# nygenome/lancet

Measured on AMD Instinct MI355X. Metric: assembled windows/sec (whole node), 600bp windows, self-tuning k, synthetic T/N, higher is better.
Workload: dtype u64; 1 GPU; chr22-scan proxy: 32768 windows/GPU x 600 bp, stride 100, 30x tumor / 30x normal, 2x150 bp, k=11..101, active-region-off; windows_per_gpu=32768, reads_per_gpu=5895305, records_rank0_contig=22477, slots_in_flight=4080, batches_in_flight=2, windows_first_graph_in_lds=32768, graphs_built_ahead=2147, graphs_taken_from_pool=2037, windows_rerun_worst_case_tier=0

## Files before the change

lancet_amd/csrc/kernels.h:

```cpp
#pragma once
#include "wave.h"
#include "layout.h"
#include "../../include/lancet_engine.h"

#ifndef LANCET_WG
#define LANCET_WG 64
#endif
#ifdef LANCET_FAT
#define LC_QLANES LC_FAT_LANES
#define LC_PF_G 6
#define LC_QSTAGE (3 * LC_FAT_LANES)
#else
#define LC_QLANES LANCET_WG
#define LC_QSTAGE LC_STAGE
#endif

enum {
  EV_PROCESS = 1, EV_REPEAT_REF, EV_NEAR_REF, EV_READS, EV_STATS, EV_MARKREF, EV_LOWCOV, EV_CLEANDEAD,
  EV_COMPRESS, EV_CC, EV_CCID, EV_CCEND, EV_TRIM, EV_AMBIG_SRC, EV_NOMATCH_SRC, EV_AMBIG_SNK, EV_NOMATCH_SNK,
  EV_CYCLE, EV_TIPS_ROUND, EV_TIPS_REMOVED, EV_LINKS, EV_LOOKREP, EV_MISSING, EV_SEARCH, EV_NEAR_QRY,
  EV_DFSLIMIT, EV_PATH, EV_TS, EV_PATH_END, EV_EKA_END, EV_FOUND, EV_END
};

struct WalkState { int nts, last_col, code; };
// ... 3596 lines not shown
      dir = dir_dest(ED_DIR(e));
    }
  }
  return len;
}
DEVNI int path_string_wg(Ctx &c, int n) {
  LC_GLOBAL Work &W = *LC_CTX(c).W; LC_WS &S = LC_SREF(c);
  const int K = S.K;
  const int dcap = 7 * ((int)LC_CTX(c).C->max_w + 2);
  if (2 * (n + 1) > dcap || n < 2) { WG_LANE0 { S.ps_len = path_string(c, n); } return wg_bcast(&S.ps_len); }
  if (n <= 64) {
    volatile LC_LDS uint8_t *lb = &S.lbytes[0];
    volatile LC_LDS uint32_t *loff = (volatile LC_LDS uint32_t *)lb, *llen = loff + 66, *lslo = llen + 64, *lshi = lslo + 64;
    volatile LC_LDS uint8_t *ldir = (volatile LC_LDS uint8_t *)(lshi + 64);
    static_assert(4 * (66 + 3 * 64) + 64 <= (int)sizeof(S.lbytes), "path nodes staged in LDS");
    WG_LANE0 { S.ps_first = 0x7FFFFFFF; }
    WG_FOR(i, n) {
      const uint32_t nd = W.pnodes[i];
      const uint32_t pe = W.pedges[i == 0 ? 1 : i];
      LC_GLOBAL const uint32_t *g = (LC_GLOBAL const uint32_t *)&W.gr[nd];
      const uint32_t fl = g[0]; const lc_u4 h1 = ldg4(g + 20);
      const uint32_t e = W.gr[pe >> 4].edges[pe & 15u];
      const bool sp = (fl & NF_SPECIAL) != 0;
      if (!sp) dev_atomic_min((LC_LDS uint32_t *)&S.ps_first, (uint32_t)i);
      ldir[i] = (uint8_t)(i == 0 ? dir_start(ED_DIR(e)) : dir_dest(ED_DIR(e)));
      lslo[i] = h1.z; lshi[i] = h1.w; llen[i] = sp ? 0xFFFFFFFFu : h1.w - h1.z;
    }
    WG_SYNC();
    const int f = wg_uniform(S.ps_first);
    WG_FOR(i, n + 1) {
      uint32_t sum = 0;
      for (int j = 0; j < i; ++j) { const uint32_t L = llen[j]; if (L != 0xFFFFFFFFu) sum += (j == f ? L : L - (uint32_t)(K - 1)); }
      loff[i] = sum;
    }
    WG_SYNC();
    const int plen = (int)wg_uniform((int)loff[n]);
    if (plen > (int)LC_CTX(c).C->path_cap) { WG_LANE0 { OVF(c); } return 0; }
    WG_FOR(x, plen) {
      int lo = 0, hi = n - 1;
      while (lo < hi) { const int mid = (lo + hi + 1) >> 1; if ((int)loff[mid] <= x) lo = mid; else hi = mid - 1; }
      while (lo > 0 && loff[lo + 1] == loff[lo]) --lo;
      const uint32_t slo = lslo[lo], shi = lshi[lo];
      const uint32_t j = (uint32_t)(x - (int)loff[lo]) + (lo == f ? 0u : (uint32_t)(K - 1));
      const uint32_t d = (ldir[lo] == (uint8_t)'R') ? (W.seq[shi - 1 - j] ^ 3u) : W.seq[slo + j];
      W.pdesc[x] = d; W.pseq[x] = (uint8_t)SD_BASE(d);
    }
    WG_SYNC();
    return plen;
  }
  LC_GLOBAL uint32_t *off = (LC_GLOBAL uint32_t *)W.dp, *pdir = off + (n + 1);
  WG_LANE0 { S.ps_first = 0x7FFFFFFF; off[n] = 0; }
  WG_FOR(i, n) {
    const uint32_t nd = W.pnodes[i];
    if (!(W.gr[nd].flags & NF_SPECIAL)) dev_atomic_min((LC_LDS uint32_t *)&S.ps_first, (uint32_t)i);
    const uint32_t pe = W.pedges[i == 0 ? 1 : i];
    const uint32_t e = W.gr[pe >> 4].edges[pe & 15u];
    pdir[i] = (uint32_t)(i == 0 ? dir_start(ED_DIR(e)) : dir_dest(ED_DIR(e)));
  }
  WG_SYNC();
  const int f = wg_uniform(S.ps_first);
  WG_FOR(i, n) {
    const uint32_t nd = W.pnodes[i];
    const int L = n_len(c, nd);
    off[i] = (W.gr[nd].flags & NF_SPECIAL) ? 0u : (uint32_t)(i == f ? L : L - (K - 1));
  }
  WG_SYNC();
  wg_scan(off, n + 1, S, S.part2);
  const int plen = (int)wg_uniform((int)S.part2[LANCET_WG]);
  if (plen > (int)LC_CTX(c).C->path_cap) { WG_LANE0 { OVF(c); } return 0; }
  WG_FOR(x, plen) {
    int lo = 0, hi = n - 1;
    while (lo < hi) { const int mid = (lo + hi + 1) >> 1; if ((int)off[mid] <= x) lo = mid; else hi = mid - 1; }
    while (lo > 0 && off[lo + 1] == off[lo]) --lo;
    const uint32_t nd = W.pnodes[lo];
    const uint32_t slo = W.gr[nd].seq_lo, shi = W.gr[nd].seq_hi;
    const uint32_t j = (uint32_t)(x - (int)off[lo]) + (lo == f ? 0u : (uint32_t)(K - 1));
    const uint32_t d = (pdir[lo] == (uint32_t)'R') ? (W.seq[shi - 1 - j] ^ 3u) : W.seq[slo + j];
    W.pdesc[x] = d; W.pseq[x] = (uint8_t)SD_BASE(d);
  }
  WG_SYNC();
  return plen;
}
DEV bool status_cnt_T(const Ctx &c, uint32_t n) {
  double pr = (double)LC_CTX(c).W->gr[n].nkmT / (double)LC_CTX(c).W->gr[n].nkm;
  return pr > 0.8;
}

#define LC_TB(i, j, n) ((size_t)((i) + (j)) * (size_t)((n) + 1) + (size_t)(i))
DEV void align_fill_arrays(Ctx &c, LC_GLOBAL const uint8_t *Sx, int n, LC_GLOBAL const uint8_t *Tx, int m) {
  LC_GLOBAL Work &W = *LC_CTX(c).W;
  const int A = (int)LC_CTX(c).C->max_w + 2;
  int32_t *Mb[3] = {W.dp, W.dp + A, W.dp + 2 * A};
  int32_t *Xb[2] = {W.dp + 3 * A, W.dp + 4 * A};
  int32_t *Yb[2] = {W.dp + 5 * A, W.dp + 6 * A};
  WG_FOR(j, m + 1) { W.tb[LC_TB(0, j, n)] = (uint8_t)((j == 0 ? 3 : 2) | (0 << 2) | (2 << 4)); }
  WG_FOR(i, n + 1) { if (i > 0) W.tb[LC_TB(i, 0, n)] = (uint8_t)(1 | (2 << 2) | (0 << 4)); }
  WG_LANE0 { Mb[0][0] = 0; Mb[1][0] = -9; Xb[1][0] = -9; Mb[1][1] = -9; Yb[1][1] = -9; }
  WG_SYNC();
  for (int d = 2; d <= n + m; ++d) {
    int32_t *Mc = Mb[d % 3], *Mp = Mb[(d + 2) % 3], *Mpp = Mb[(d + 1) % 3];
    int32_t *Xc = Xb[d & 1], *Xp = Xb[(d + 1) & 1], *Yc = Yb[d & 1], *Yp = Yb[(d + 1) & 1];
    int ilo = d - m; if (ilo < 1) ilo = 1;
    int ihi = d - 1; if (ihi > n) ihi = n;
    WG_FOR(t, ihi - ilo + 1) {
      int i = ilo + t, j = d - i;
      int xa = Xp[i - 1] + (-1), xb = Mp[i - 1] + (-8);
      int xs, xt; if (xa > xb) { xs = xa; xt = 1; } else { xs = xb; xt = 0; }
      int ya = Yp[i] + (-1), yb = Mp[i] + (-8);
      int ys, yt; if (ya > yb) { ys = ya; yt = 1; } else { ys = yb; yt = 0; }
      int ms = Mpp[i - 1] + (Sx[i - 1] == Tx[j - 1] ? 2 : -4), mt = 0;
      if (xs > ms) { ms = xs; mt = 1; }
      if (ys > ms) { ms = ys; mt = 2; }
      Mc[i] = ms; Xc[i] = xs; Yc[i] = ys;
      W.tb[LC_TB(i, j, n)] = (uint8_t)(mt | (xt << 2) | (yt << 4));
    }
    WG_LANE0 {
      if (d <= m) { Mc[0] = -8 - d; Xc[0] = -8 - d; }
      if (d <= n) { Mc[d] = -8 - d; Yc[d] = -8 - d; }
    }
    WG_SYNC();
  }
}
#ifndef LANCET_WAVE_EMU
template <int GMAX>
DEVNI void align_fill_g(Ctx &c, LC_GLOBAL const uint8_t *Sx, int n, LC_GLOBAL const uint8_t *Tx, int m) {
  static_assert(LANCET_WG == 64, "one wave per window");
  LC_GLOBAL Work &W = *LC_CTX(c).W;
  if (threadIdx.x == 0) LC_SREF(c).al_band = 0;
  const int lane = (int)threadIdx.x;
  if (lane < 64) {
  for (int j = lane; j < m + 1; j += 64) W.tb[LC_TB(0, j, n)] = (uint8_t)((j == 0 ? 3 : 2) | (0 << 2) | (2 << 4));
  for (int i = lane + 1; i < n + 1; i += 64) W.tb[LC_TB(i, 0, n)] = (uint8_t)(1 | (2 << 2) | (0 << 4));
  const int G = (n + 63) / 64;
  int A[GMAX], Bv[GMAX], sg[GMAX];
  auto lo16 = [](int v) -> int { return (int)(short)(v & 0xFFFF); };
  auto hi16 = [](int v) -> int { return v >> 16; };
  auto pack = [](int lo, int hi) -> int { return (lo & 0xFFFF) | (hi << 16); };
#pragma unroll
  for (int g = 0; g < GMAX; ++g) {
    int i = g * 64 + lane + 1;
    A[g] = pack(-8 - i, 0);
    Bv[g] = pack(-8 - i, (i - 1 == 0) ? 0 : -8 - (i - 1));
    sg[g] = (i <= n) ? (int)Sx[i - 1] : 255;
  }
  for (int t = 2; t <= n + m; ++t) {
#pragma unroll
    for (int gg = 0; gg < GMAX; ++gg) {
      const int g = GMAX - 1 - gg;
      if (g < G) {
        int i = g * 64 + lane + 1, j = t - i;
        int nb = __shfl_up(A[g], 1);
        if (g > 0) { int e = __shfl(A[g > 0 ? g - 1 : 0], 63); if (lane == 0) nb = e; }
        else if (lane == 0) nb = pack(-8 - j, -8 - j);
        int nbM = lo16(nb), nbX = hi16(nb);
        bool active = (i <= n) && (j >= 1) && (j <= m);
        int bv = Bv[g];
        if (active) {
          int xa = nbX - 1, xb = nbM - 8;
          int xs, xt; if (xa > xb) { xs = xa; xt = 1; } else { xs = xb; xt = 0; }
          int ya = lo16(bv) - 1, yb = lo16(A[g]) - 8;
          int ys, yt; if (ya > yb) { ys = ya; yt = 1; } else { ys = yb; yt = 0; }
          int ms = hi16(bv) + (sg[g] == (int)Tx[j - 1] ? 2 : -4), mt = 0;
          if (xs > ms) { ms = xs; mt = 1; }
          if (ys > ms) { ms = ys; mt = 2; }
          A[g] = pack(ms, xs);
          bv = pack(ys, hi16(bv));
          W.tb[LC_TB(i, j, n)] = (uint8_t)(mt | (xt << 2) | (yt << 4));
        }
        if (j >= 1) bv = pack(lo16(bv), nbM);
        Bv[g] = bv;
      }
    }
  }
  }
  WG_SYNC();
}
DEV void align_fill(Ctx &c, LC_GLOBAL const uint8_t *Sx, int n, LC_GLOBAL const uint8_t *Tx, int m) {
  if (n <= LC_MAXW_DEFAULT) { align_fill_g<(LC_MAXW_DEFAULT + 63) / 64>(c, Sx, n, Tx, m); return; }
  WG_LANE0 { LC_SREF(c).al_band = 0; }
  align_fill_arrays(c, Sx, n, Tx, m);
}
#else
DEV void align_fill(Ctx &c, LC_GLOBAL const uint8_t *Sx, int n, LC_GLOBAL const uint8_t *Tx, int m) { LC_SREF(c).al_band = 0; align_fill_arrays(c, Sx, n, Tx, m); }
#endif
#define LC_BNEG (-(1 << 24))
template <bool B> struct LcBool { static constexpr bool value = B; };
DEV void band_cell(int i, int j, int sch, int tch, int dM, int uM, int uX, int lM, int lY, int *oM, int *oX, int *oY, uint8_t *otb) {
  const int xa = uX - 1, xb = uM - 8;
  int xs, xt; if (xa > xb) { xs = xa; xt = 1; } else { xs = xb; xt = 0; }
  const int ya = lY - 1, yb = lM - 8;
  int ys, yt; if (ya > yb) { ys = ya; yt = 1; } else { ys = yb; yt = 0; }
  int ms = dM + (sch == tch ? 2 : -4), mt = 0;
  if (xs > ms) { ms = xs; mt = 1; }
  if (ys > ms) { ms = ys; mt = 2; }
  (void)i; (void)j;
  *oM = ms; *oX = xs; *oY = ys; *otb = (uint8_t)(mt | (xt << 2) | (yt << 4));
}
DEVNI bool align_fill_band(Ctx &c, LC_GLOBAL const uint8_t *Sx, int n, LC_GLOBAL const uint8_t *Tx, int m) {
  LC_GLOBAL Work &W = *LC_CTX(c).W; LC_WS &S = LC_SREF(c);
  const int d = m - n;
  const int w = (127 - (d < 0 ? -d : d)) / 2;
  if (w < 8 || n < 1 || m < 1) return false;
  const int lo = (d < 0 ? d : 0) - w, hi = lo + 127;
  if ((size_t)(n + m + 2) * 64 > (size_t)(LC_CTX(c).C->max_w + LC_CTX(c).C->path_cap + 4) * (LC_CTX(c).C->max_w + 2)) return false;
  WG_LANE0 { S.al_band = 1; S.al_lo = lo; S.al_score = LC_BNEG; }
#ifndef LANCET_WAVE_EMU
  {
    const int lane = (int)threadIdx.x;
    LC_GLOBAL uint8_t *tbp = W.tb;
    int ME = LC_BNEG, XE = LC_BNEG, YE = LC_BNEG, MO = LC_BNEG, XO = LC_BNEG, YO = LC_BNEG;
    int fin = LC_BNEG;
    LC_LDS uint8_t *ls = (LC_LDS uint8_t *)&S.lbytes[0];
    const bool staged = (size_t)(n + m) <= sizeof(S.lbytes);
    if (staged) { WG_FOR(x, n) { ls[x] = Sx[x]; } WG_FOR(x, m) { ls[n + x] = Tx[x]; } }
    WG_SYNC();
    auto run = [&](auto STG) {
      constexpr bool stg = decltype(STG)::value;
      const int oE = lo + 2 * lane, oO = oE + 1;
      const bool okE = oE <= hi, okO = oO <= hi;
      auto cell = [&](const int t, const int o, const bool ok, const int dM0, const int uM0, const int uX0, const int lM0, const int lY0, int &oM, int &oX, int &oY) {
        const int i = (t - o) >> 1, j = t - i;
        const bool valid = ok && i >= 1 && i <= n && j >= 1 && j <= m;
        int dM = dM0, uM = uM0, uX = uX0, lM = lM0, lY = lY0;
        if (i == 1) { uM = -8 - j; uX = -8 - j; dM = (j == 1) ? 0 : -8 - (j - 1); }
        if (j == 1) { lM = -8 - i; lY = -8 - i; if (i != 1) dM = -8 - (i - 1); }
        const int ic = valid ? i - 1 : 0, jc = valid ? j - 1 : 0;
        int sch, tch;
        if constexpr (stg) { sch = (int)ls[ic]; tch = (int)ls[n + jc]; } else { sch = (int)Sx[ic]; tch = (int)Tx[jc]; }
        const int xa = uX - 1, xb = uM - 8;
        const int xs = xa > xb ? xa : xb, xt = xa > xb ? 1 : 0;
        const int ya = lY - 1, yb = lM - 8;
        const int ys = ya > yb ? ya : yb, yt = ya > yb ? 1 : 0;
        int ms = dM + (sch == tch ? 2 : -4), mt = 0;
        if (xs > ms) { ms = xs; mt = 1; }
        if (ys > ms) { ms = ys; mt = 2; }
        if (valid) {
          tbp[(size_t)t * 64 + (size_t)lane] = (uint8_t)(mt | (xt << 2) | (yt << 4));
          if (i == n && j == m) fin = ms;
        }
        oM = valid ? ms : LC_BNEG; oX = valid ? xs : LC_BNEG; oY = valid ? ys : LC_BNEG;
      };
      auto stepE = [&](const int t) {
        const int lM = __builtin_amdgcn_update_dpp(LC_BNEG, MO, 0x138, 0xf, 0xf, false);
        const int lY = __builtin_amdgcn_update_dpp(LC_BNEG, YO, 0x138, 0xf, 0xf, false);
        int cM, cX, cY; cell(t, oE, okE, ME, MO, XO, lM, lY, cM, cX, cY);
        ME = cM; XE = cX; YE = cY;
      };
      auto stepO = [&](const int t) {
        const int uM = __builtin_amdgcn_update_dpp(LC_BNEG, ME, 0x130, 0xf, 0xf, false);
        const int uX = __builtin_amdgcn_update_dpp(LC_BNEG, XE, 0x130, 0xf, 0xf, false);
        int cM, cX, cY; cell(t, oO, okO, MO, uM, uX, ME, YE, cM, cX, cY);
        MO = cM; XO = cX; YO = cY;
      };
      int t = 2;
      if (((t - lo) & 1) != 0) { stepO(t); ++t; }
      for (; t + 1 <= n + m; t += 2) { stepE(t); stepO(t + 1); }
      if (t <= n + m) stepE(t);
    };
    if (lane < 64) { if (staged) run(LcBool<true>{}); else run(LcBool<false>{}); }
    if (fin != LC_BNEG) S.al_score = fin;
  }
#else
  {
    int M1[64], X1[64], Y1[64], M2[64];
    for (int l = 0; l < 64; ++l) { M1[l] = X1[l] = Y1[l] = M2[l] = LC_BNEG; }
    for (int t = 2; t <= n + m; ++t) {
      const int pt = (t - lo) & 1;
      int nM_[64], nX_[64], nY_[64];
      for (int lane = 0; lane < 64; ++lane) {
        const int o = lo + 2 * lane + pt;
        const int i = (t - o) >> 1, j = t - i;
        const bool valid = o <= hi && i >= 1 && i <= n && j >= 1 && j <= m;
        const int nl = pt ? lane + 1 : lane - 1;
        int nM = (nl < 0 || nl > 63) ? LC_BNEG : M1[nl];
        int nXY = (nl < 0 || nl > 63) ? LC_BNEG : (pt ? X1[nl] : Y1[nl]);
        int uM = pt ? nM : M1[lane], uX = pt ? nXY : X1[lane];
        int lM = pt ? M1[lane] : nM, lY = pt ? Y1[lane] : nXY;
        int dM = M2[lane];
        if (i == 1) { uM = -8 - j; uX = -8 - j; dM = (j == 1) ? 0 : -8 - (j - 1); }
        if (j == 1) { lM = -8 - i; lY = -8 - i; if (i != 1) dM = -8 - (i - 1); }
        int cM = LC_BNEG, cX = LC_BNEG, cY = LC_BNEG; uint8_t tb = 0;
        if (valid) {
          band_cell(i, j, (int)Sx[i - 1], (int)Tx[j - 1], dM, uM, uX, lM, lY, &cM, &cX, &cY, &tb);
          W.tb[(size_t)t * 64 + (size_t)lane] = tb;
          if (i == n && j == m) S.al_score = cM;
        }
        nM_[lane] = cM; nX_[lane] = cX; nY_[lane] = cY;
      }
      for (int l = 0; l < 64; ++l) { M2[l] = M1[l]; M1[l] = nM_[l]; X1[l] = nX_[l]; Y1[l] = nY_[l]; }
    }
  }
#endif
  WG_SYNC();
  const int score = wg_bcast(&S.al_score);
  const int gh = hi + 1, gv_h = hi + 1 - d;
  const int gv = 1 - lo, gh_l = 1 - lo + d;
  const int out_hi = 2 * (m - gh) - (7 + gh) - (7 + gv_h);
  const int out_lo = 2 * (n - gv) - (7 + gv) - (7 + gh_l);
  const int bound = out_hi > out_lo ? out_hi : out_lo;
  if (score == LC_BNEG || score <= bound) { WG_LANE0 { S.al_band = 0; } return false; }
  return true;
}

DEVNI int align_traceback(Ctx &c, LC_GLOBAL const uint8_t *Sx, int n, LC_GLOBAL const uint8_t *Tx, int m) {
  LC_GLOBAL Work &W = *LC_CTX(c).W;
  const int cap = (int)LC_CTX(c).C->max_w + (int)LC_CTX(c).C->path_cap + 2;
  LC_GLOBAL uint32_t *cols = W.scratch;
  (void)Sx; (void)Tx;
  int i = n, j = m, L = 0;
  bool forcex = false, forcey = false;
  unsigned long long pre = 0; int bi = -1, bj = -1, used = 8;
  while (i > 0 || j > 0) {
    if (i < 0 || j < 0 || L >= cap) { OVF(c); return 0; }
    if (used >= 8 || i != bi - used || j != bj - used) {
      bi = i; bj = j; used = 0;
      pre = 0;
      if (!LC_SREF(c).al_band) { for (int q = 0; q < 8; ++q) pre |= (unsigned long long)((i - q >= 0 && j - q >= 0) ? W.tb[LC_TB(i - q, j - q, n)] : (uint8_t)0) << (8 * q); }
      else {
        const int blo = LC_SREF(c).al_lo;
        for (int q = 0; q < 8; ++q) {
          const int ii = i - q, jj = j - q;
          uint8_t bb = 0;
          if (ii >= 0 && jj >= 0) {
            if (ii == 0) bb = (uint8_t)((jj == 0 ? 3 : 2) | (0 << 2) | (2 << 4));
            else if (jj == 0) bb = (uint8_t)(1 | (2 << 2) | (0 << 4));
            else { const int tt = ii + jj, oo = jj - ii; bb = W.tb[(size_t)tt * 64 + (size_t)((oo - blo - ((tt - blo) & 1)) >> 1)]; }
          }
          pre |= (unsigned long long)bb << (8 * q);
        }
      }
    }
    uint8_t b = (uint8_t)(pre >> (8 * used)); ++used;
    int t = b & 3, x = (b >> 2) & 3, y = (b >> 4) & 3;
    if (t == 3) break;
    else if (forcex) { if (i < 1) { OVF(c); return 0; } cols[L++] = ((uint32_t)i << 16) | ((uint32_t)j << 2) | 1u; if (x == 0) forcex = false; --i; }
    else if (t == 1) { cols[L++] = ((uint32_t)i << 16) | ((uint32_t)j << 2) | 1u; if (x == 1) forcex = true; --i; }
    else if (forcey) { if (j < 1) { OVF(c); return 0; } cols[L++] = ((uint32_t)i << 16) | ((uint32_t)j << 2) | 2u; if (y == 0) forcey = false; --j; }
    else if (t == 2) { cols[L++] = ((uint32_t)i << 16) | ((uint32_t)j << 2) | 2u; if (y == 1) forcey = true; --j; }
    else { cols[L++] = ((uint32_t)i << 16) | ((uint32_t)j << 2); --i; --j; }
  }
  return L;
}
DEVNI int align_traceback_wg(Ctx &c, LC_GLOBAL const uint8_t *Sx, int n, LC_GLOBAL const uint8_t *Tx, int m) {
  LC_WS &S = LC_SREF(c);
#ifdef LANCET_WAVE_EMU
  WG_LANE0 { S.al_L = align_traceback(c, Sx, n, Tx, m); }
  return wg_bcast(&S.al_L);
#else
  LC_GLOBAL Work &W = *LC_CTX(c).W;
  (void)Sx; (void)Tx;
  if (threadIdx.x < 64) {
    const int lane = (int)threadIdx.x;
    const int cap = (int)LC_CTX(c).C->max_w + (int)LC_CTX(c).C->path_cap + 2;
    LC_GLOBAL uint32_t *cols = W.scratch;
    LC_GLOBAL const uint8_t *tbp = W.tb;
    const int band = S.al_band, blo = S.al_lo;
    int i = n, j = m, L = 0;
    bool forcex = false, forcey = false, bad = false;
    int ci = 0, cj = 0, cdir = -1;
    uint32_t mine = 0, note = 0;
    while (i > 0 || j > 0) {
      if (i < 0 || j < 0 || L >= cap) { bad = true; break; }
      const int want = forcex ? 1 : (forcey ? 2 : 0);
      int q = -1;
      if (cdir == want) {
        if (want == 0) { if (ci - i == cj - j) q = ci - i; }
        else if (want == 1) { if (cj == j) q = ci - i; }
        else { if (ci == i) q = cj - j; }
      }
      if (q < 0 || q > 63) {
        cdir = want; ci = i; cj = j; q = 0;
        const int ii = want == 2 ? i : i - lane, jj = want == 1 ? j : j - lane;
        uint32_t bb = 0;
        if (ii >= 0 && jj >= 0) {
          if (!band) bb = tbp[LC_TB(ii, jj, n)];
          else if (ii == 0) bb = (uint32_t)((jj == 0 ? 3 : 2) | (0 << 2) | (2 << 4));
          else if (jj == 0) bb = (uint32_t)(1 | (2 << 2) | (0 << 4));
          else { const int tt = ii + jj, oo = jj - ii; const int li = (oo - blo - ((tt - blo) & 1)) >> 1; bb = (li >= 0 && li < 64) ? tbp[(size_t)tt * 64 + (size_t)li] : 0u; }
        }
        mine = bb;
      }
      const uint32_t b = (uint32_t)__shfl((int)mine, q, 64);
      const int t = (int)(b & 3u), x = (int)((b >> 2) & 3u), y = (int)((b >> 4) & 3u);
      uint32_t v;
      if (t == 3) break;
      else if (forcex) { if (i < 1) { bad = true; break; } v = ((uint32_t)i << 16) | ((uint32_t)j << 2) | 1u; if (x == 0) forcex = false; --i; }
      else if (t == 1) { v = ((uint32_t)i << 16) | ((uint32_t)j << 2) | 1u; if (x == 1) forcex = true; --i; }
      else if (forcey) { if (j < 1) { bad = true; break; } v = ((uint32_t)i << 16) | ((uint32_t)j << 2) | 2u; if (y == 0) forcey = false; --j; }
      else if (t == 2) { v = ((uint32_t)i << 16) | ((uint32_t)j << 2) | 2u; if (y == 1) forcey = true; --j; }
      else { v = ((uint32_t)i << 16) | ((uint32_t)j << 2); --i; --j; }
      if (lane == (L & 63)) note = v;
      ++L;
      if ((L & 63) == 0) cols[L - 64 + lane] = note;
    }
    if (!bad && lane < (L & 63)) cols[(L & ~63) + lane] = note;
    if (lane == 0) { if (bad) { OVF(c); L = 0; } S.al_L = L; }
  }
  return wg_bcast(&S.al_L);
#endif
}
#define LC_NOTE_JMAX 0x3FFF
DEVNI void align_traceback_fill(Ctx &c, LC_GLOBAL const uint8_t *Sx, LC_GLOBAL const uint8_t *Tx, int L) {
  LC_GLOBAL Work &W = *LC_CTX(c).W;
  const int cap = (int)LC_CTX(c).C->max_w + (int)LC_CTX(c).C->path_cap + 2;
  LC_GLOBAL uint8_t *ra = W.aln, *pa = W.aln + cap;
  LC_GLOBAL const uint32_t *cols = W.scratch;
  WG_FOR(x, L) {
    const uint32_t v = cols[L - 1 - x];
    const int i = (int)(v >> 16), j = (int)((v >> 2) & 0x3FFFu), kind = (int)(v & 3u);
    ra[x] = kind == 2 ? (uint8_t)'-' : (uint8_t)"ACGTN"[Sx[i - 1]];
    pa[x] = kind == 1 ? (uint8_t)'-' : (uint8_t)"ACGT"[Tx[j - 1]];
  }
  WG_SYNC();
}

#ifndef LANCET_WAVE_EMU
DEV void align_test_body(const EngineCaps *C, Work *work, const uint8_t *Sx, int n, const uint8_t *Tx, int m, int *out_len, int mode) {
  LC_WS &S = *(LC_WS *)&lc_shared;
  Ctx c; c.P = nullptr; c.B = nullptr; c.C = (LC_GLOBAL const EngineCaps *)C; c.W = (LC_GLOBAL Work *)work; c.OUT = nullptr; c.S = &S;
  LC_CTX_PUBLISH(c);
  WG_LANE0 { S.overflow = 0; }
  WG_SYNC();
  if (mode == 1 || !align_fill_band(c, (LC_GLOBAL const uint8_t *)Sx, n, (LC_GLOBAL const uint8_t *)Tx, m)) {
    if (mode == 2) { WG_LANE0 { *out_len = -2; } return; }
    align_fill(c, (LC_GLOBAL const uint8_t *)Sx, n, (LC_GLOBAL const uint8_t *)Tx, m);
  }
  { const int L = align_traceback_wg(c, (LC_GLOBAL const uint8_t *)Sx, n, (LC_GLOBAL const uint8_t *)Tx, m); WG_LANE0 { S.tmp0 = L; *out_len = S.overflow ? -1 : L; } }
  align_traceback_fill(c, (LC_GLOBAL const uint8_t *)Sx, (LC_GLOBAL const uint8_t *)Tx, wg_bcast(&S.tmp0));
}
#endif

struct Acc {
  uint16_t first, mn, mnz, sum, sumnz, nnz; uint32_t n;
};
template <class A> DEV void acc_init(A &a, uint16_t v) { a.first = v; a.mn = v; a.mnz = v; a.sum = 0; a.sumnz = 0; a.nnz = 0; a.n = 0; a.sum = (uint16_t)(a.sum + v); if (v != 0) { a.sumnz = (uint16_t)(a.sumnz + v); ++a.nnz; } a.n = 1; }
template <class A> DEV void acc_push(A &a, uint16_t v) {
  a.sum = (uint16_t)(a.sum + v); if (v != 0) { a.sumnz = (uint16_t)(a.sumnz + v); a.nnz = (uint16_t)(a.nnz + 1); }
  if (v < a.mn) a.mn = v;
  if (v < a.mnz && v != 0) a.mnz = v;
  ++a.n;
}
template <class A> DEV uint16_t acc_mean(const A &a) { return a.n > 0 ? (uint16_t)((float)a.sum / (float)a.n) : (uint16_t)0; }

struct TS {
  uint32_t pos, ref_pos, start_pos, end_pos, ref_end_pos;
  int col0, col1;
  char code, prev_bp_ref, prev_bp_alt; bool somatic;
  Acc aN[4], aT[4], rN[2], rT[2];
  uint16_t hrmnN[3], hrmnT[3], hrsumN[3], hrsumT[3], hamnN[3], hamnT[3], haqN[3], haqT[3];
};
constexpr int LC_TS_LDS = (int)(sizeof(WinShared::lbytes) / sizeof(TS));
struct TSHead { uint32_t pos, ref_pos, start_pos, end_pos, ref_end_pos; int col0, col1; char code, prev_bp_ref, prev_bp_alt; };
struct HPc { uint16_t nh[3], nq[3], th[3], tq[3]; };
template <class T> DEV void ts_hp_init(T &t, const HPc &a, const HPc &r) {
  for (int j = 0; j < 3; ++j) {
    t.hrmnN[j] = r.nh[j]; t.hrmnT[j] = r.th[j]; t.hrsumN[j] = r.nh[j]; t.hrsumT[j] = r.th[j];
    t.hamnN[j] = a.nh[j]; t.hamnT[j] = a.th[j]; t.haqN[j] = a.nq[j]; t.haqT[j] = a.tq[j];
  }
}
template <class T> DEV void ts_hp_add_alt(T &t, const HPc &a) {
  for (int j = 0; j < 3; ++j) {
    if (a.nh[j] < t.hamnN[j]) t.hamnN[j] = a.nh[j];
    if (a.th[j] < t.hamnT[j]) t.hamnT[j] = a.th[j];
    if (a.nq[j] < t.haqN[j]) t.haqN[j] = a.nq[j];
    if (a.tq[j] < t.haqT[j]) t.haqT[j] = a.tq[j];
  }
}
template <class T> DEV void ts_hp_add_ref(T &t, const HPc &r) {
  for (int j = 0; j < 3; ++j) {
    if (r.nh[j] < t.hrmnN[j]) t.hrmnN[j] = r.nh[j];
    if (r.th[j] < t.hrmnT[j]) t.hrmnT[j] = r.th[j];
    t.hrsumN[j] = (uint16_t)(t.hrsumN[j] + r.nh[j]); t.hrsumT[j] = (uint16_t)(t.hrsumT[j] + r.th[j]);
  }
}
DEV void ref_hp_at(const Ctx &c, uint32_t pos, HPc &r) {
  for (int j = 0; j < 3; ++j) { r.nh[j] = r.th[j] = r.nq[j] = r.tq[j] = 0; }
  if (!LC_SREF(c).LR || (int)pos >= LC_SREF(c).reflen) return;
  const uint16_t *h = LC_CTX(c).W->refhp + 6 * pos;
  for (int j = 0; j < 3; ++j) { r.th[j] = h[j]; r.nh[j] = h[3 + j]; }
}
DEV void path_hp_at(const Ctx &c, int P, HPc &a) {
  for (int j = 0; j < 3; ++j) { a.nh[j] = a.th[j] = a.nq[j] = a.tq[j] = 0; }
  if (!LC_SREF(c).LR) return;
  uint32_t d = LC_CTX(c).W->pdesc[P];
  desc_hp(c, d, 0, a.nh, a.nq);
  desc_hp(c, d, 1, a.th, a.tq);
}
template <class T> DEV void ts_add_alt(T &t, const uint16_t *n4, const uint16_t *t4) { for (int q = 0; q < 4; ++q) { acc_push(t.aN[q], n4[q]); acc_push(t.aT[q], t4[q]); } }
template <class T> DEV void ts_add_ref(T &t, const uint16_t *n2, const uint16_t *t2) { for (int q = 0; q < 2; ++q) { acc_push(t.rN[q], n2[q]); acc_push(t.rT[q], t2[q]); } }

DEV void ref_cov_at(const Ctx &c, uint32_t pos, uint16_t *n2, uint16_t *t2) {
  if ((int)pos < LC_SREF(c).reflen) { const uint16_t *r = LC_CTX(c).W->refcov + 4 * pos; t2[0] = r[0]; t2[1] = r[1]; n2[0] = r[2]; n2[1] = r[3]; }
  else { n2[0] = n2[1] = t2[0] = t2[1] = 0; }
}
DEV void path_cov_at(const Ctx &c, int P, uint16_t *n4, uint16_t *t4) {
  uint32_t d = LC_CTX(c).W->pdesc[P];
  desc_cov(c, d, 0, &n4[0], &n4[1], &n4[2], &n4[3]);
  desc_cov(c, d, 1, &t4[0], &t4[1], &t4[2], &t4[3]);
}

DEV void bx_add_node(Ctx &c, uint32_t X, uint32_t nml, uint32_t *n) {
  LC_GLOBAL Work &W = *LC_CTX(c).W; LC_GLOBAL const DevBatch &B = *LC_CTX(c).B; LC_WS &S = LC_SREF(c);
  const uint32_t g0 = B.read_begin[S.w], refr = (uint32_t)(S.R - 1);
  LC_GLOBAL uint32_t *buf = W.bxbuf;
  for (uint32_t i = W.nocc[X]; i < W.nocc[X + 1]; ++i) {
    const uint32_t r = CS_READ(W_CSR(W)[i]);
    if (r == refr) continue;
    if (RI_NML(B.rinfo[g0 + r]) != nml) continue;
    const uint32_t bx = B.bx_rank[g0 + r];
    if (bx == 0xFFFFFFFFu) continue;
    uint32_t lo = 0, hi = *n;
    while (lo < hi) { uint32_t mid = (lo + hi) >> 1; if (buf[mid] < bx) lo = mid + 1; else hi = mid; }
    if (lo < *n && buf[lo] == bx) continue;
    if (*n >= LC_CTX(c).C->reads_cap) { OVF(c); return; }
    for (uint32_t j = *n; j > lo; --j) buf[j] = buf[j - 1];
    buf[lo] = bx; ++*n;
  }
}
DEVNI uint32_t kmer_lookup(Ctx &c, const uint8_t *codes, int *ori) {
  LC_GLOBAL Work &W = *LC_CTX(c).W; LC_WS &S = LC_SREF(c);
  const int K = S.K, NW = S.NW;
  unsigned long long fw[LC_NWMAX], rc[LC_NWMAX];
  for (int w = 0; w < LC_NWMAX; ++w) { fw[w] = 0; rc[w] = 0; }
  for (int i = 0; i < K; ++i) { key_push_fw(fw, NW, K, codes[i] & 3); key_push_rc(rc, NW, K, codes[i] & 3); }
  const unsigned long long *ck = key_less(fw, rc, NW) ? fw : rc;
  if (ori) *ori = ck == fw ? 0 : (key_less(rc, fw, NW) ? 1 : 2);
  const uint32_t mask = S.tmask;
  unsigned long long h = 0; uint32_t idx;
  if (NW == 1 && K <= 31) { h = ck[0] + 1ULL; idx = (uint32_t)mix64(h) & mask; }
  else {
    for (int w = 0; w < NW; ++w) h = mix64(h ^ (ck[w] + 0x9e3779b97f4a7c15ULL * (unsigned long long)(w + 1)));
    h &= ~(1ULL << 63);
    if (h == 0) h = 1;
    idx = (uint32_t)h & mask;
  }
  for (uint32_t probes = 0; probes <= mask; ++probes) {
    const unsigned long long cur = SL_TAG(W, idx);
    if (cur == 0) return LC_NIL;
    if (cur == h) {
      bool same = true;
      if (!(NW == 1 && K <= 31)) for (int w = 0; w < NW; ++w) if (W.slot_key[(size_t)idx * LC_NWMAX + w] != ck[w]) same = false;
      if (same) return SL_NODE(W, idx);
    }
    idx = (idx + 1) & mask;
  }
  return LC_NIL;
}
DEVNI void emit_variant_lr(Ctx &c, uint32_t vi, const TSHead &t, const uint16_t hp12[12], int plen) {
  LC_WS &S = LC_SREF(c); LC_GLOBAL Work &W = *LC_CTX(c).W; DevOut &O = *LC_CTX(c).OUT;
  lancet_variant_lr &l = O.variants_lr[vi];
  for (int q = 0; q < 12; ++q) l.hp[q] = hp12[q];
  l.reserved[0] = l.reserved[1] = 0;
  const int K = S.K;
  const uint32_t ro = W.occ_base[S.R - 1];
  for (int q = 0; q < 4; ++q) {
    const uint32_t nml = (q == 0 || q == 2) ? 1u : 0u;
    uint32_t n = 0;
    if (q < 2) {
      for (int i = (int)t.ref_pos - 1; i <= (int)t.ref_end_pos - 1; ++i) {
        if (i < 0 || i + K > S.seq_len) continue;
        const uint32_t rv = S.prebuilt ? W.lr_refnode[S.seq_t5 + i] : 0u;
        const uint32_t X = S.prebuilt ? (rv & 0x3FFFFFFFu) : (W.occ[ro + (uint32_t)(S.seq_t5 + i)] & 0x3FFFFFFFu);
        if (S.prebuilt ? (rv >> 31) != 0u : (W.gr[X].flags & NF_INMER) != 0u) bx_add_node(c, X, nml, &n);
      }
    } else {
      for (int i = (int)t.start_pos - 2; i <= (int)t.end_pos - 1; ++i) {
        if (i < 0 || i + K > plen) continue;
        const uint32_t X = kmer_lookup(c, W.pseq + i);
        if (X != LC_NIL) bx_add_node(c, X, nml, &n);
      }
    }
    const uint32_t off = dev_atomic_add(O.n_bx, n);
    if (off + n > LC_CTX(c).C->bx_cap) { OVF(c); l.bx_off[q] = 0; l.bx_len[q] = 0; continue; }
    l.bx_off[q] = off; l.bx_len[q] = n;
    for (uint32_t j = 0; j < n; ++j) O.bx_blob[off + j] = W.bxbuf[j];
  }
}

DEVNI void emit_variant(Ctx &c, const TSHead &t, const uint16_t cov[8], int strLen, const uint8_t *motif, int motifLen, bool hasStr,
                      const uint8_t *ra, const uint8_t *pa, const uint16_t hp12[12], int plen) {
  LC_WS &S = LC_SREF(c); DevOut &O = *LC_CTX(c).OUT;
  uint32_t vi = dev_atomic_add(O.n_variants, 1u);
  int rl = t.col1 - t.col0 + 1;
  char sbuf[80]; int sl = 0;
  if (hasStr) {
    char digs[12]; int nd = 0; int v = strLen; do { digs[nd++] = (char)('0' + v % 10); v /= 10; } while (v);
    while (nd) sbuf[sl++] = digs[--nd];
    for (int i = 0; i < motifLen; ++i) sbuf[sl++] = "ACGT"[motif[i]];
  }
  uint32_t need = (uint32_t)(2 * rl + sl);
  uint32_t bo = dev_atomic_add(O.n_blob, need);
  if (vi >= LC_CTX(c).C->var_cap || bo + need > LC_CTX(c).C->blob_cap) { OVF(c); return; }
  lancet_variant &v = O.variants[vi];
  v.window = S.w; v.seq_in_window = S.emit_seq++; v.chr_id = LC_CTX(c).B->chr_id[S.w]; v.pos = (int32_t)t.pos - 1;
  v.code = (uint8_t)t.code; v.prev_bp_ref = (uint8_t)t.prev_bp_ref; v.prev_bp_alt = (uint8_t)t.prev_bp_alt; v.reserved = 0;
  v.kmer = (uint16_t)S.K; for (int q = 0; q < 8; ++q) v.cov[q] = cov[q]; v.reserved2 = 0;
  v.ref_off = bo; v.ref_len = (uint32_t)rl; v.alt_off = bo + (uint32_t)rl; v.alt_len = (uint32_t)rl; v.str_off = bo + 2u * (uint32_t)rl; v.str_len = (uint32_t)sl;
  for (int i = 0; i < rl; ++i) { O.blob[bo + i] = (char)ra[t.col0 + i]; O.blob[bo + rl + i] = (char)pa[t.col0 + i]; }
  for (int i = 0; i < sl; ++i) O.blob[bo + 2 * rl + i] = sbuf[i];
  if (S.LR) emit_variant_lr(c, vi, t, hp12, plen);
}

DEVNI void walk_prepare(Ctx &c, int L) {
  LC_WS &S = LC_SREF(c); LC_GLOBAL Work &W = *LC_CTX(c).W;
  const int cap = (int)LC_CTX(c).C->max_w + (int)LC_CTX(c).C->path_cap + 2;
  LC_GLOBAL const uint8_t *ra = W.aln, *pa = W.aln + cap;
  LC_GLOBAL uint32_t *E1 = W.scratch, *E2 = W.scratch + (L + 1), *F = W.scratch + 2 * (L + 1), *cols = W.scratch + 3 * (L + 1);
  WG_LANE0 { S.wk[0] = S.wk[1] = S.wk[2] = S.wk[3] = 0; E1[L] = 0; E2[L] = 0; F[L] = 0; }
  WG_FOR(i, L) {
    const uint8_t r = ra[i], p = pa[i];
    E1[i] = r != '-'; E2[i] = p != '-'; F[i] = r != p;
    const int t = r == p ? 0 : (r == '-' ? 2 : (p == '-' ? 3 : 1));
    dev_atomic_add((LC_LDS uint32_t *)&S.wk[t], 1u);
  }
  WG_SYNC();
  wg_scan(E1, L + 1, S, S.part2);
  wg_scan(E2, L + 1, S, S.part2);
  wg_scan(F, L + 1, S, S.part2);
  WG_FOR(i, L) { if (F[i + 1] != F[i]) cols[F[i]] = (uint32_t)i; }
  WG_LANE0 { S.wk_n = (int)F[L]; }
}
#define LC_HD_MAX 5
DEVNI void walk_prepare_unaligned(Ctx &c, int L, int hd) {
  LC_WS &S = LC_SREF(c); LC_GLOBAL Work &W = *LC_CTX(c).W;
  LC_GLOBAL uint32_t *E1 = W.scratch, *E2 = W.scratch + (L + 1), *cols = W.scratch + 3 * (L + 1);
  WG_LANE0 {
    for (int a = 1; a < hd; ++a) {
      const uint32_t v = S.part2[a]; int b = a;
      for (; b > 0 && S.part2[b - 1] > v; --b) S.part2[b] = S.part2[b - 1];
      S.part2[b] = v;
    }
    for (int a = 0; a < hd; ++a) { const uint32_t i = S.part2[a]; cols[a] = i; E1[i] = i; E2[i] = i; }
    S.wk[0] = L - hd; S.wk[1] = hd; S.wk[2] = 0; S.wk[3] = 0; S.wk_n = hd;
  }
}
DEVNI void process_path_perfect_wg(Ctx &c, int np, int n, int complete) {
  LC_WS &S = LC_SREF(c); LC_GLOBAL Work &W = *LC_CTX(c).W;
  WG_LANE0 {
    evt(c, EV_PATH, (uint32_t)complete, (uint32_t)S.tmp3, (uint32_t)n, 0u, 0u, 0u);
    evt(c, EV_PATH_END);
    ++S.tmp0;
  }
  WG_FOR(i, np) { dev_atomic_add(&W.gr[W.pnodes[i]].onref, 1u); }
}

struct WalkPos {
  uint16_t cn4[4], ct4[4], rn2[2], rt2[2];
  HPc ha, hr;
  int col, P; uint32_t pos_in_ref; char code;
  bool tumor, no_spanner, p_outside;
};
enum { WALK_GO = 0, WALK_END = 1, WALK_OVF = 2, WALK_FULL = 3 };
DEV WalkState walk_state_load(LC_WS &S) { WalkState st; st.nts = S.wk_st.nts; st.last_col = S.wk_st.last_col; st.code = S.wk_st.code; return st; }
DEV void walk_state_store(LC_WS &S, const WalkState &st) { S.wk_st.nts = st.nts; S.wk_st.last_col = st.last_col; S.wk_st.code = st.code; }
DEV void hp_zero(HPc &h) { for (int j = 0; j < 3; ++j) { h.nh[j] = h.th[j] = h.nq[j] = h.tq[j] = 0; } }
DEV char column_code(uint8_t r, uint8_t p) { return r == '-' ? '^' : (p == '-' ? 'v' : 'x'); }
DEV void walk_pos_load(Ctx &c, WalkPos &v, int P, uint32_t refpos, int plen, bool lr) {
  v.P = P; v.p_outside = P < 0 || P >= plen;
  for (int q = 0; q < 4; ++q) { v.cn4[q] = 0; v.ct4[q] = 0; }
  hp_zero(v.ha); hp_zero(v.hr);
  if (!v.p_outside) { path_cov_at(c, P, v.cn4, v.ct4); if (lr) path_hp_at(c, P, v.ha); }
  ref_cov_at(c, refpos, v.rn2, v.rt2);
  if (lr) ref_hp_at(c, refpos, v.hr);
}
template <class TP> DEV int walk_column(Ctx &c, TP ts, WalkState &st, int cap, const WalkPos &v, LC_GLOBAL const uint8_t *ra, LC_GLOBAL const uint8_t *pa, unsigned rrpos, bool lr) {
  const char prev_code = (st.last_col == v.col - 1) ? (char)st.code : '=';
  const char code = v.code;
  st.last_col = v.col; st.code = (int)code;
  if (v.no_spanner) return WALK_END;
  if (v.p_outside) { OVF(c); return WALK_OVF; }
  if (st.nts > 0 && prev_code != '=') {
    auto &t = ts[st.nts - 1];
    if (v.tumor) t.somatic = true;
    const bool del_next = t.pos + (unsigned)(t.col1 - t.col0 + 1) + 1u == rrpos;
    t.col1 = v.col; t.end_pos = (uint32_t)v.P; t.ref_end_pos = v.pos_in_ref;
    if (code == '^' && t.code == code && t.pos == rrpos) { ts_add_alt(t, v.cn4, v.ct4); if (lr) ts_hp_add_alt(t, v.ha); }
    else if (code == 'v' && t.code == code && del_next) { ts_add_ref(t, v.rn2, v.rt2); if (lr) ts_hp_add_ref(t, v.hr); }
    else if (code == 'x' || t.code != code) { t.code = 'c'; ts_add_alt(t, v.cn4, v.ct4); ts_add_ref(t, v.rn2, v.rt2); if (lr) { ts_hp_add_alt(t, v.ha); ts_hp_add_ref(t, v.hr); } }
    return WALK_GO;
  }
  int pr = v.col - 1, pq = v.col - 1;
  while (pr >= 0 && ra[pr] != 'A' && ra[pr] != 'C' && ra[pr] != 'G' && ra[pr] != 'T') --pr;
  while (pq >= 0 && pa[pq] != 'A' && pa[pq] != 'C' && pa[pq] != 'G' && pa[pq] != 'T') --pq;
  if (pr < 0 || pq < 0) { OVF(c); return WALK_OVF; }
  if (st.nts >= LC_MAXTS) { OVF(c); return WALK_OVF; }
  if (st.nts >= cap) return WALK_FULL;
  auto &t = ts[st.nts++];
  t.pos = rrpos; t.ref_pos = v.pos_in_ref; t.start_pos = (uint32_t)(v.P + 1); t.code = code; t.end_pos = (uint32_t)v.P; t.ref_end_pos = v.pos_in_ref;
  t.col0 = v.col; t.col1 = v.col; t.somatic = v.tumor; t.prev_bp_ref = (char)ra[pr]; t.prev_bp_alt = (char)pa[pq];
  for (int q = 0; q < 4; ++q) { acc_init(t.aN[q], v.cn4[q]); acc_init(t.aT[q], v.ct4[q]); }
  for (int q = 0; q < 2; ++q) { acc_init(t.rN[q], v.rn2[q]); acc_init(t.rT[q], v.rt2[q]); }
  ts_hp_init(t, v.ha, v.hr);
  return WALK_GO;
}
template <class T> DEV bool walk_extend(T &t, const WalkPos &v, bool lr) {
  if (!v.p_outside) {
    if (v.no_spanner) return false;
    if (v.tumor) t.somatic = true;
    ts_add_alt(t, v.cn4, v.ct4); if (lr) ts_hp_add_alt(t, v.ha);
  }
  ts_add_ref(t, v.rn2, v.rt2); if (lr) ts_hp_add_ref(t, v.hr);
  return true;
// ... 1076 lines not shown
```

Measured before the change: 892,100 windows/s.

## Emit alignment traceback in ballot-detected runs instead of cell by cell

The wave-level alignment traceback now loads a 64-cell line of traceback bytes, uses a ballot to find where the current move (diagonal, forced-x or forced-y) stops, and writes the whole run of column entries in parallel across lanes. Only cells that change state go through the serial per-step decoder. Previously every cell needed a shuffle plus serial branching. The intent is to cut the serial per-cell latency of traceback. In exchange the code adds ballot and ctz work, scattered per-run stores, and a getenv fallback to the old path in emulation builds.

```diff
diff --git a/lancet_amd/csrc/kernels.h b/lancet_amd/csrc/kernels.h
--- a/lancet_amd/csrc/kernels.h
+++ b/lancet_amd/csrc/kernels.h
@@ -3922,7 +3922,8 @@
   return true;
 }
 
-DEVNI int align_traceback(Ctx &c, LC_GLOBAL const uint8_t *Sx, int n, LC_GLOBAL const uint8_t *Tx, int m) {
+#ifdef LANCET_WAVE_EMU
+DEVNI int align_traceback_cells(Ctx &c, LC_GLOBAL const uint8_t *Sx, int n, LC_GLOBAL const uint8_t *Tx, int m) {
   LC_GLOBAL Work &W = *LC_CTX(c).W;
   const int cap = (int)LC_CTX(c).C->max_w + (int)LC_CTX(c).C->path_cap + 2;
   LC_GLOBAL uint32_t *cols = W.scratch;
@@ -3961,63 +3962,105 @@
   }
   return L;
 }
+#endif
+DEV uint32_t align_tb_byte(LC_GLOBAL const uint8_t *tbp, int band, int blo, int n, int ii, int jj) {
+  if (ii < 0 || jj < 0) return 0u;
+  if (!band) return tbp[LC_TB(ii, jj, n)];
+  if (ii == 0) return (uint32_t)((jj == 0 ? 3 : 2) | (0 << 2) | (2 << 4));
+  if (jj == 0) return (uint32_t)(1 | (2 << 2) | (0 << 4));
+  const int tt = ii + jj, oo = jj - ii, li = (oo - blo - ((tt - blo) & 1)) >> 1;
+  return (li >= 0 && li < 64) ? tbp[(size_t)tt * 64 + (size_t)li] : 0u;
+}
+#ifndef LANCET_WAVE_EMU
+struct TbLine {
+  uint32_t v;
+  template <class F> DEVM void fetch(F cell) { v = cell((int)threadIdx.x); }
+  template <class P> DEVM unsigned long long stops(P stop) const { return __ballot(stop((int)threadIdx.x, v) ? 1 : 0); }
+  DEVM uint32_t at(int q) const { return (uint32_t)__builtin_amdgcn_readlane((int)v, lc_sgpr(q)); }
+};
+#define TB_EACH_LANE(l) for (int l = (int)threadIdx.x, l##_once = 1; l##_once; l##_once = 0)
+#else
+struct TbLine {
+  uint32_t v[64];
+  template <class F> DEVM void fetch(F cell) { for (int l = 0; l < 64; ++l) v[l] = cell(l); }
+  template <class P> DEVM unsigned long long stops(P stop) const { unsigned long long s = 0; for (int l = 0; l < 64; ++l) { if (stop(l, v[l])) s |= 1ULL << l; } return s; }
+  DEVM uint32_t at(int q) const { return v[q]; }
+};
+#define TB_EACH_LANE(l) for (int l = 0; l < 64; ++l)
+#endif
+DEV int align_traceback_runs(Ctx &c, int n, int m) {
+  LC_GLOBAL Work &W = *LC_CTX(c).W; LC_WS &S = LC_SREF(c);
+  const int cap = lc_sgpr((int)LC_CTX(c).C->max_w + (int)LC_CTX(c).C->path_cap + 2);
+  LC_GLOBAL uint32_t *cols = W.scratch;
+  LC_GLOBAL const uint8_t *tbp = W.tb;
+  const int band = lc_sgpr((int)S.al_band), blo = lc_sgpr((int)S.al_lo);
+  n = lc_sgpr(n); m = lc_sgpr(m);
+  int i = n, j = m, L = 0;
+  bool forcex = false, forcey = false;
+  int ci = 0, cj = 0, cdir = -1;
+  unsigned long long stop = 0;
+  TbLine line;
+  while (i > 0 || j > 0) {
+    if (i < 0 || j < 0 || L >= cap) return -1;
+    const int want = forcex ? 1 : (forcey ? 2 : 0);
+    int q = -1;
+    if (cdir == want) {
+      if (want == 0) { if (ci - i == cj - j) q = ci - i; }
+      else if (want == 1) { if (cj == j) q = ci - i; }
+      else { if (ci == i) q = cj - j; }
+    }
+    if (q < 0 || q > 63) {
+      cdir = want; ci = i; cj = j; q = 0;
+      line.fetch([&](int l) { return align_tb_byte(tbp, band, blo, n, want == 2 ? i : i - l, want == 1 ? j : j - l); });
+      stop = line.stops([&](int l, uint32_t b) {
+        if (want == 0) return (b & 3u) != 0u || i - l < 0 || j - l < 0;
+        if (want == 1) return ((b >> 2) & 3u) == 0u || (b & 3u) == 3u || i - l < 1;
+        return ((b >> 4) & 3u) == 0u || (b & 1u) != 0u || j - l < 1;
+      });
+    }
+    const unsigned long long rem = stop >> q;
+    int r = rem ? (int)__builtin_ctzll(rem) : 64 - q;
+    if (r > cap - L) r = cap - L;
+    if (r > 0) {
+      const int di = want == 2 ? 0 : 1, dj = want == 1 ? 0 : 1;
+      TB_EACH_LANE(l) { const int x = l - q; if (x >= 0 && x < r) cols[L + x] = ((uint32_t)(i - x * di) << 16) | ((uint32_t)(j - x * dj) << 2) | (uint32_t)want; }
+      i -= r * di; j -= r * dj; L += r;
+      continue;
+    }
+    const uint32_t b = line.at(q);
+    const int t = (int)(b & 3u), x = (int)((b >> 2) & 3u), y = (int)((b >> 4) & 3u);
+    uint32_t v;
+    if (t == 3) break;
+    else if (forcex) { if (i < 1) return -1; v = ((uint32_t)i << 16) | ((uint32_t)j << 2) | 1u; if (x == 0) forcex = false; --i; }
+    else if (t == 1) { v = ((uint32_t)i << 16) | ((uint32_t)j << 2) | 1u; if (x == 1) forcex = true; --i; }
+    else if (forcey) { if (j < 1) return -1; v = ((uint32_t)i << 16) | ((uint32_t)j << 2) | 2u; if (y == 0) forcey = false; --j; }
+    else if (t == 2) { v = ((uint32_t)i << 16) | ((uint32_t)j << 2) | 2u; if (y == 1) forcey = true; --j; }
+    else { v = ((uint32_t)i << 16) | ((uint32_t)j << 2); --i; --j; }
+    TB_EACH_LANE(l) { if (l == q) cols[L] = v; }
+    ++L;
+  }
+  return L;
+}
+#ifdef LANCET_WAVE_EMU
+DEVNI int align_traceback(Ctx &c, LC_GLOBAL const uint8_t *Sx, int n, LC_GLOBAL const uint8_t *Tx, int m) {
+  if (getenv("LANCET_OLD_TRACEBACK") != nullptr) return align_traceback_cells(c, Sx, n, Tx, m);
+  const int L = align_traceback_runs(c, n, m);
+  if (L < 0) { OVF(c); return 0; }
+  return L;
+}
+#endif
 DEVNI int align_traceback_wg(Ctx &c, LC_GLOBAL const uint8_t *Sx, int n, LC_GLOBAL const uint8_t *Tx, int m) {
   LC_WS &S = LC_SREF(c);
 #ifdef LANCET_WAVE_EMU
   WG_LANE0 { S.al_L = align_traceback(c, Sx, n, Tx, m); }
-  return wg_bcast(&S.al_L);
 #else
-  LC_GLOBAL Work &W = *LC_CTX(c).W;
   (void)Sx; (void)Tx;
   if (threadIdx.x < 64) {
-    const int lane = (int)threadIdx.x;
-    const int cap = (int)LC_CTX(c).C->max_w + (int)LC_CTX(c).C->path_cap + 2;
-    LC_GLOBAL uint32_t *cols = W.scratch;
-    LC_GLOBAL const uint8_t *tbp = W.tb;
-    const int band = S.al_band, blo = S.al_lo;
-    int i = n, j = m, L = 0;
-    bool forcex = false, forcey = false, bad = false;
-    int ci = 0, cj = 0, cdir = -1;
-    uint32_t mine = 0, note = 0;
-    while (i > 0 || j > 0) {
-      if (i < 0 || j < 0 || L >= cap) { bad = true; break; }
-      const int want = forcex ? 1 : (forcey ? 2 : 0);
-      int q = -1;
-      if (cdir == want) {
-        if (want == 0) { if (ci - i == cj - j) q = ci - i; }
-        else if (want == 1) { if (cj == j) q = ci - i; }
-        else { if (ci == i) q = cj - j; }
-      }
-      if (q < 0 || q > 63) {
-        cdir = want; ci = i; cj = j; q = 0;
-        const int ii = want == 2 ? i : i - lane, jj = want == 1 ? j : j - lane;
-        uint32_t bb = 0;
-        if (ii >= 0 && jj >= 0) {
-          if (!band) bb = tbp[LC_TB(ii, jj, n)];
-          else if (ii == 0) bb = (uint32_t)((jj == 0 ? 3 : 2) | (0 << 2) | (2 << 4));
-          else if (jj == 0) bb = (uint32_t)(1 | (2 << 2) | (0 << 4));
-          else { const int tt = ii + jj, oo = jj - ii; const int li = (oo - blo - ((tt - blo) & 1)) >> 1; bb = (li >= 0 && li < 64) ? tbp[(size_t)tt * 64 + (size_t)li] : 0u; }
-        }
-        mine = bb;
-      }
-      const uint32_t b = (uint32_t)__shfl((int)mine, q, 64);
-      const int t = (int)(b & 3u), x = (int)((b >> 2) & 3u), y = (int)((b >> 4) & 3u);
-      uint32_t v;
-      if (t == 3) break;
-      else if (forcex) { if (i < 1) { bad = true; break; } v = ((uint32_t)i << 16) | ((uint32_t)j << 2) | 1u; if (x == 0) forcex = false; --i; }
-      else if (t == 1) { v = ((uint32_t)i << 16) | ((uint32_t)j << 2) | 1u; if (x == 1) forcex = true; --i; }
-      else if (forcey) { if (j < 1) { bad = true; break; } v = ((uint32_t)i << 16) | ((uint32_t)j << 2) | 2u; if (y == 0) forcey = false; --j; }
-      else if (t == 2) { v = ((uint32_t)i << 16) | ((uint32_t)j << 2) | 2u; if (y == 1) forcey = true; --j; }
-      else { v = ((uint32_t)i << 16) | ((uint32_t)j << 2); --i; --j; }
-      if (lane == (L & 63)) note = v;
-      ++L;
-      if ((L & 63) == 0) cols[L - 64 + lane] = note;
-    }
-    if (!bad && lane < (L & 63)) cols[(L & ~63) + lane] = note;
-    if (lane == 0) { if (bad) { OVF(c); L = 0; } S.al_L = L; }
-  }
+    int L = align_traceback_runs(c, n, m);
+    if (threadIdx.x == 0) { if (L < 0) { OVF(c); L = 0; } S.al_L = L; }
+  }
+#endif
   return wg_bcast(&S.al_L);
-#endif
 }
 #define LC_NOTE_JMAX 0x3FFF
 DEVNI void align_traceback_fill(Ctx &c, LC_GLOBAL const uint8_t *Sx, LC_GLOBAL const uint8_t *Tx, int L) {
```

New measurement: 903,400 windows/s, median of 6. 1.01x the previous value.
